# okieraised/rs-face-detection-tflite

Measured on AMD Instinct MI355X. Metric: faces/sec at batch=256 (256x256 back-camera) per GPU, higher is better.
Workload: dtype f32

## Files before the change

rs-face-detection-tflite_amd/csrc/mstrip_kernels.hip:

```cpp
#include <hip/hip_runtime.h>

#include <algorithm>
#include <cstdint>
#include <cstdio>
#include <cstdlib>
#include <type_traits>
#include <utility>

#include "kernels.hpp"
#include "launch.hpp"
#include "wave_sync.hpp"

namespace mi {

namespace {

typedef float v2f __attribute__((ext_vector_type(2)));
typedef float f32x4 __attribute__((ext_vector_type(4)));

struct MstripArgs {
    const float* in;
    float* out;
    const float* consts;
    long in_fs, out_fs;
    int B, H;
    int bands, band_rows;
    int has_res;
    float hi;
    unsigned long long* stamps;
};

constexpr int kMstripChain = 8;
struct MstripChainArgs {
    const float* in[kMstripChain];
    float* out[kMstripChain];
    const float* consts[kMstripChain];
    long in_fs[kMstripChain], out_fs[kMstripChain];
    int has_res[kMstripChain];
    float hi[kMstripChain];
    int nblocks, B, H;
};

template <int CK>
struct MK {
    static constexpr int C = 4 * CK, MT = C / 16;
    static constexpr int QP = CK + 1;
    static constexpr int PS = 4 * QP;
    static constexpr int IMG_F = 34 * PS;
    static constexpr int DPX = 64 / QP;
    static constexpr int NLD = 32 / DPX;
    static_assert(32 % DPX == 0 && NLD == 8, "eight DMA instructions per row (two source bases, four immediate offsets each)");
    static_assert((16 * PS) % 64 == 0 && 16 * PS / 64 < 256, "ds_read2st64_b32 reaches the second pixel tile");
    static constexpr int OFF_A = 0, A_F = CK * MT * 64, OFF_TAP = A_F, TAP_F = CK * 48, OFF_BIAS = OFF_TAP + TAP_F, OFF_SLOPE = OFF_BIAS + C, TOTAL = OFF_SLOPE + C;
    static constexpr int WG_F = A_F + 2 * C + TAP_F;
    static constexpr int NBUF = 2;
};

template <class F, int... KS>
__device__ __forceinline__ void mfor_each(F&& f, std::integer_sequence<int, KS...>) { (f(std::integral_constant<int, KS>{}), ...); }

template <int CK, bool RELU>
__global__ __launch_bounds__(256, 2) void mstrip_kernel(MstripArgs a) {
    using K = MK<CK>;
    constexpr int C = K::C, MT = K::MT, PS = K::PS, QP = K::QP, IMG_F = K::IMG_F, NLD = K::NLD, NBUF = K::NBUF;
    extern __shared__ __attribute__((aligned(16))) float lds[];
#ifdef MI_MSTRIP_STAMPS
    unsigned long long st_acc[7] = {0, 0, 0, 0, 0, 0, 0}, st_prev = __builtin_amdgcn_s_memtime();
#define MI_MSTAMP(k) { __builtin_amdgcn_sched_barrier(0); unsigned long long t_ = __builtin_amdgcn_s_memtime(); asm volatile("s_waitcnt lgkmcnt(0)" ::: "memory"); st_acc[k] += t_ - st_prev; st_prev = t_; __builtin_amdgcn_sched_barrier(0); }
#else
#define MI_MSTAMP(k)
#endif
    const int lane = threadIdx.x & 63;
    const int wave = __builtin_amdgcn_readfirstlane(threadIdx.x >> 6);
    const int kq = lane >> 4, p = lane & 15;
    float* wgc = lds;
    float* img = lds + K::WG_F + wave * NBUF * IMG_F;
    const int unit = blockIdx.x * 4 + wave;
    const int band = unit / a.B, b = unit - band * a.B;
    const bool active = band < a.bands;
    const int y0 = band * a.band_rows, y1 = min(y0 + a.band_rows, a.H);
    const float* in = a.in + (long)b * a.in_fs;

    const int goff = ((lane / QP) * C + 4 * min(lane % QP, CK - 1)) * 4;
    const unsigned lds_img = __builtin_amdgcn_readfirstlane((unsigned)(uintptr_t)(__attribute__((address_space(3))) float*)img);
    auto issue_row = [&](int r, int bi) {
        const char* src = reinterpret_cast<const char*>(in + (long)min(max(r, 0), a.H - 1) * 32 * C);
        const char* src1 = src + (NLD / 2) * K::DPX * C * 4;
        const unsigned dstb = lds_img + (unsigned)((bi * IMG_F + PS) * 4);
        constexpr int ACTIVE = K::DPX * QP;
        static_assert(ACTIVE > 32 && ACTIVE < 64, "exec mask written as two 32-bit halves");
        unsigned long long saved;
#define MI_MS_DMA(base, k) "s_add_u32 m0, m0, %7\n\ts_nop 0\n\tglobal_load_lds_dwordx4 %3, " base " offset:" #k "*%8\n\t"
        asm volatile("s_mov_b64 %0, exec\n\ts_mov_b32 exec_lo, -1\n\ts_mov_b32 exec_hi, %6\n\t"
                     "s_mov_b32 m0, %4\n\ts_nop 0\n\tglobal_load_lds_dwordx4 %3, %1\n\t"
                     MI_MS_DMA("%1", 1) MI_MS_DMA("%1", 2) MI_MS_DMA("%1", 3)
                     "s_add_u32 m0, m0, %5\n\ts_nop 0\n\tglobal_load_lds_dwordx4 %3, %2\n\t"
                     MI_MS_DMA("%2", 1) MI_MS_DMA("%2", 2) MI_MS_DMA("%2", 3)
                     "s_mov_b64 exec, %0"
                     : "=&s"(saved)
                     : "s"(src), "s"(src1), "v"(goff), "s"(dstb), "n"((NLD / 2) * K::DPX * PS * 4 - (NLD / 2 - 1) * K::DPX * (PS - C) * 4),
                       "n"((1u << (ACTIVE - 32)) - 1), "n"(K::DPX * (PS - C) * 4), "n"(K::DPX * C * 4)
                     : "memory", "scc", "m0");
#undef MI_MS_DMA
    };
    auto fix_row = [&](int r, int bi) {
        if (r >= 0 && r < a.H) return;
        float zz = 0.f;
        asm volatile("" : "+v"(zz));
        const float4 z = make_float4(zz, zz, zz, zz);
        float* part = img + bi * IMG_F + PS;
        constexpr int N4 = 32 * QP;
#pragma unroll
        for (int k = 0; k < (N4 + 63) / 64; k++)
            if (64 * (k + 1) <= N4 || lane < N4 - 64 * k) *reinterpret_cast<float4*>(part + 4 * (lane + 64 * k)) = z;
    };
    if (lane < 2 * QP) {
        const int col = lane / QP, qd = lane - col * QP;
#pragma unroll
        for (int bi = 0; bi < NBUF; bi++) *reinterpret_cast<float4*>(img + bi * IMG_F + col * 33 * PS + 4 * qd) = make_float4(0.f, 0.f, 0.f, 0.f);
    }

    if (active) issue_row(y0 - 1, 0);
    MI_MSTAMP(5)
    for (int i = threadIdx.x; i < K::A_F / 4; i += 256) reinterpret_cast<float4*>(wgc)[i] = reinterpret_cast<const float4*>(a.consts + K::OFF_A)[i];
    for (int i = threadIdx.x; i < 2 * C; i += 256) wgc[K::A_F + i] = a.consts[K::OFF_BIAS + i];
    for (int i = threadIdx.x; i < K::TAP_F / 4; i += 256) reinterpret_cast<float4*>(wgc + K::A_F + 2 * C)[i] = reinterpret_cast<const float4*>(a.consts + K::OFF_TAP)[i];
    if (active) issue_row(y0, 1);
    if (active) wait_vm<NLD>(); else wait_vm<0>();
    MI_MSTAMP(6)
    asm volatile("s_waitcnt lgkmcnt(0)" ::: "memory");
    __builtin_amdgcn_s_barrier();
    asm volatile("" ::: "memory");
    float tap[CK][9];
    {
        const float4* tp = reinterpret_cast<const float4*>(wgc + K::A_F + 2 * C) + kq * 3;
#pragma unroll
        for (int ks = 0; ks < CK; ks++) {
            const float4 t0 = tp[ks * 12], t1 = tp[ks * 12 + 1], t2 = tp[ks * 12 + 2];
            tap[ks][0] = t0.x; tap[ks][1] = t0.y; tap[ks][2] = t0.z; tap[ks][3] = t0.w;
            tap[ks][4] = t1.x; tap[ks][5] = t1.y; tap[ks][6] = t1.z; tap[ks][7] = t1.w;
            tap[ks][8] = t2.x;
        }
#pragma unroll
        for (int ks = 0; ks < CK; ks++)
#pragma unroll
            for (int t = 0; t < 9; t++) asm volatile("" : "+v"(tap[ks][t]));
    }
    if (!active) return;
    MI_MSTAMP(0)
    const float* xme = img + p * PS + kq;
    const float* sme = img + (1 + p) * PS + 4 * kq;
    const float* ame = wgc + lane;
    const unsigned ooff = (unsigned)(p * C + 4 * kq) * 4u;

    float accA[CK][2], accB[CK][2];
    f32x4 D[MT][2];
#pragma unroll
    for (int ks = 0; ks < CK; ks++) accA[ks][0] = accA[ks][1] = accB[ks][0] = accB[ks][1] = 0.f;

    auto init_D = [&](int bi) {
        float4 bs[MT], x[MT][2];
#pragma unroll
        for (int mt = 0; mt < MT; mt++) bs[mt] = *reinterpret_cast<const float4*>(wgc + K::A_F + 16 * mt + 4 * kq);
        if (a.has_res) {
#pragma unroll
            for (int mt = 0; mt < MT; mt++)
#pragma unroll
                for (int nt = 0; nt < 2; nt++) x[mt][nt] = *reinterpret_cast<const float4*>(sme + bi * IMG_F + 16 * nt * PS + 16 * mt);
#pragma unroll
            for (int mt = 0; mt < MT; mt++)
#pragma unroll
                for (int nt = 0; nt < 2; nt++) D[mt][nt] = f32x4{x[mt][nt].x + bs[mt].x, x[mt][nt].y + bs[mt].y, x[mt][nt].z + bs[mt].z, x[mt][nt].w + bs[mt].w};
        } else {
#pragma unroll
            for (int mt = 0; mt < MT; mt++) D[mt][0] = D[mt][1] = f32x4{bs[mt].x, bs[mt].y, bs[mt].z, bs[mt].w};
        }
    };
    typedef __attribute__((address_space(1))) char gchar;
    typedef __attribute__((address_space(1))) f32x4 gf32x4;
    auto epilogue = [&](int y) {
        gchar* dst = (gchar*)(a.out + (long)b * a.out_fs + (long)y * 32 * C);
        asm volatile("" : "+s"(dst));
#pragma unroll
        for (int mt = 0; mt < MT; mt++) {
            float4 sl = make_float4(0.f, 0.f, 0.f, 0.f);
            if (!RELU) sl = *reinterpret_cast<const float4*>(wgc + K::A_F + C + 16 * mt + 4 * kq);
#pragma unroll
            for (int nt = 0; nt < 2; nt++) {
                f32x4 v = D[mt][nt];
                if (RELU) {
                    v = f32x4{fmaxf(v.x, 0.f), fmaxf(v.y, 0.f), fmaxf(v.z, 0.f), fmaxf(v.w, 0.f)};
                } else {
                    v = f32x4{fminf(fmaxf(v.x, 0.f) + sl.x * fminf(v.x, 0.f), a.hi), fminf(fmaxf(v.y, 0.f) + sl.y * fminf(v.y, 0.f), a.hi),
                              fminf(fmaxf(v.z, 0.f) + sl.z * fminf(v.z, 0.f), a.hi), fminf(fmaxf(v.w, 0.f) + sl.w * fminf(v.w, 0.f), a.hi)};
                }
                *(gf32x4*)(dst + ooff + (unsigned)((16 * nt * C + 16 * mt) * 4)) = v;
            }
        }
    };

    const unsigned x_lds = (unsigned)(uintptr_t)(__attribute__((address_space(3))) float*)const_cast<float*>(xme);
    const unsigned a_lds = (unsigned)(uintptr_t)(__attribute__((address_space(3))) float*)const_cast<float*>(ame);
    auto row = [&](auto emit, int bi, float (&aPN)[CK][2], float (&aC)[CK][2]) {
        constexpr bool EMIT = decltype(emit)::value;
        const unsigned xr = x_lds + (unsigned)(bi * IMG_F * 4), ar = a_lds;
        float xs[2][3][2], av[2][MT];
        auto load_ks = [&](auto ksc, float (&x)[3][2], float (&aw)[MT]) {
            constexpr int ks = decltype(ksc)::value;
            const unsigned xa = xr, aa = ar;
#pragma unroll
            for (int dx = 0; dx < 3; dx++) {
                asm volatile("ds_read_b32 %0, %1 offset:%2" : "=v"(x[dx][0]) : "v"(xa), "n"((dx * PS + 4 * ks) * 4));
                asm volatile("ds_read_b32 %0, %1 offset:%2" : "=v"(x[dx][1]) : "v"(xa), "n"((dx * PS + 4 * ks + 16 * PS) * 4));
            }
            if constexpr (EMIT) {
#pragma unroll
                for (int mt = 0; mt < MT; mt++) asm volatile("ds_read_b32 %0, %1 offset:%2" : "=v"(aw[mt]) : "v"(aa), "n"((ks * MT + mt) * 64 * 4));
            }
        };
        auto landed = [&](float (&x)[3][2], float (&aw)[MT]) {
#pragma unroll
            for (int dx = 0; dx < 3; dx++) asm volatile("" : "+v"(x[dx][0]), "+v"(x[dx][1]));
            if constexpr (EMIT) {
#pragma unroll
                for (int mt = 0; mt < MT; mt++) asm volatile("" : "+v"(aw[mt]));
            }
        };
        auto kstep = [&](auto ksc) {
            constexpr int ks = decltype(ksc)::value;
            if constexpr (ks + 1 < CK) load_ks(std::integral_constant<int, ks + 1>{}, xs[(ks + 1) & 1], av[(ks + 1) & 1]);
            float (&x)[3][2] = xs[ks & 1];
            float (&aw)[MT] = av[ks & 1];
            const float (&w)[9] = tap[ks];
            float pch[2];
#pragma unroll
            for (int nt = 0; nt < 2; nt++) {
                float n = x[0][nt] * w[0], c = aC[ks][nt], pc = aPN[ks][nt];
#pragma unroll
                for (int dx = 0; dx < 3; dx++) {
                    if (EMIT) pc = __builtin_fmaf(x[dx][nt], w[6 + dx], pc);
                    if (dx) n = __builtin_fmaf(x[dx][nt], w[dx], n);
                    c = __builtin_fmaf(x[dx][nt], w[3 + dx], c);
                }
                aC[ks][nt] = c;
                aPN[ks][nt] = n;
                asm volatile("" : "+v"(aC[ks][nt]), "+v"(aPN[ks][nt]));
                pch[nt] = pc;
            }
            if constexpr (EMIT) {
#pragma unroll
                for (int mt = 0; mt < MT; mt++) {
                    D[mt][0] = __builtin_amdgcn_mfma_f32_16x16x4f32(aw[mt], pch[0], D[mt][0], 0, 0, 0);
                    D[mt][1] = __builtin_amdgcn_mfma_f32_16x16x4f32(aw[mt], pch[1], D[mt][1], 0, 0, 0);
                }
            }
            asm volatile("s_waitcnt lgkmcnt(0)" ::: "memory");
            if constexpr (ks + 1 < CK) landed(xs[(ks + 1) & 1], av[(ks + 1) & 1]);
            __builtin_amdgcn_sched_barrier(0);
        };
        load_ks(std::integral_constant<int, 0>{}, xs[0], av[0]);
        asm volatile("s_waitcnt lgkmcnt(0)" ::: "memory");
        landed(xs[0], av[0]);
        __builtin_amdgcn_sched_barrier(0);
        mfor_each(kstep, std::make_integer_sequence<int, CK>{});
    };

    constexpr int NST = 2 * MT;
    auto wait_row = [&](int t) {
        const bool st = t - 1 >= 2, dm = t == 0 || (t - 1) + 2 <= (y1 - y0 + 1);
        if (st && dm) wait_vm<NST + NLD>();
        else if (dm) wait_vm<NLD>();
        else if (st) wait_vm<NST>();
        else wait_vm<0>();
    };
    auto step = [&](auto emit, int r, float (&aPN)[CK][2], float (&aC)[CK][2]) {
        const int t = r - (y0 - 1), bi = t & 1;
        wait_row(t);
        fix_row(r, bi);
        wave_sync();
        MI_MSTAMP(1)
        row(emit, bi, aPN, aC);
        MI_MSTAMP(2)
        __builtin_amdgcn_sched_barrier(0);
        if constexpr (decltype(emit)::value) epilogue(r - 1);
        MI_MSTAMP(3)
        __builtin_amdgcn_sched_barrier(0);
        init_D(bi);
        __builtin_amdgcn_sched_barrier(0);
        wave_sync();
        __builtin_amdgcn_s_waitcnt(0xC07F);
        if (r + 2 <= y1) issue_row(r + 2, bi);
        MI_MSTAMP(4)
    };
    step(std::false_type{}, y0 - 1, accA, accB);
    step(std::false_type{}, y0, accB, accA);
    for (int r = y0 + 1; r <= y1; r += 2) {
        step(std::true_type{}, r, accA, accB);
        if (r + 1 > y1) break;
        step(std::true_type{}, r + 1, accB, accA);
    }
#ifdef MI_MSTRIP_STAMPS
    if (a.stamps && lane == 0)
        for (int k = 0; k < 7; k++) a.stamps[(long)unit * 8 + k] = st_acc[k];
#endif
}

template <int CK, bool RELU>
__global__ __launch_bounds__(512, 2) void mstrip_chain_kernel(MstripChainArgs ca) {
    using K = MK<CK>;
    constexpr int C = K::C, MT = K::MT, PS = K::PS, QP = K::QP, IMG_F = K::IMG_F, NLD = K::NLD, NBUF = K::NBUF;
    extern __shared__ __attribute__((aligned(16))) float lds[];
#ifdef MI_MSTRIP_STAMPS
    unsigned long long st_acc[7] = {0, 0, 0, 0, 0, 0, 0}, st_prev = __builtin_amdgcn_s_memtime();
#define MI_MSTAMP(k) { __builtin_amdgcn_sched_barrier(0); unsigned long long t_ = __builtin_amdgcn_s_memtime(); asm volatile("s_waitcnt lgkmcnt(0)" ::: "memory"); st_acc[k] += t_ - st_prev; st_prev = t_; __builtin_amdgcn_sched_barrier(0); }
#else
#define MI_MSTAMP(k)
#endif
    const int lane = threadIdx.x & 63;
    const int wave = __builtin_amdgcn_readfirstlane(threadIdx.x >> 6);
    const int kq = lane >> 4, p = lane & 15;
    float* img = lds + 2 * K::WG_F + wave * NBUF * IMG_F;
    const int b = blockIdx.x;
    const int y0 = 4 * wave, y1 = y0 + 4;
    struct { int H; } a{ca.H};
    const float* in = nullptr;
    float* wgc = lds;

    const int goff = ((lane / QP) * C + 4 * min(lane % QP, CK - 1)) * 4;
    const unsigned lds_img = __builtin_amdgcn_readfirstlane((unsigned)(uintptr_t)(__attribute__((address_space(3))) float*)img);
    auto issue_row = [&](int r, int bi) {
        const char* src = reinterpret_cast<const char*>(in + (long)min(max(r, 0), a.H - 1) * 32 * C);
        const char* src1 = src + (NLD / 2) * K::DPX * C * 4;
        const unsigned dstb = lds_img + (unsigned)((bi * IMG_F + PS) * 4);
        constexpr int ACTIVE = K::DPX * QP;
        static_assert(ACTIVE > 32 && ACTIVE < 64, "exec mask written as two 32-bit halves");
        unsigned long long saved;
#define MI_MS_DMA(base, k) "s_add_u32 m0, m0, %7\n\ts_nop 0\n\tglobal_load_lds_dwordx4 %3, " base " offset:" #k "*%8\n\t"
        asm volatile("s_mov_b64 %0, exec\n\ts_mov_b32 exec_lo, -1\n\ts_mov_b32 exec_hi, %6\n\t"
                     "s_mov_b32 m0, %4\n\ts_nop 0\n\tglobal_load_lds_dwordx4 %3, %1\n\t"
                     MI_MS_DMA("%1", 1) MI_MS_DMA("%1", 2) MI_MS_DMA("%1", 3)
                     "s_add_u32 m0, m0, %5\n\ts_nop 0\n\tglobal_load_lds_dwordx4 %3, %2\n\t"
                     MI_MS_DMA("%2", 1) MI_MS_DMA("%2", 2) MI_MS_DMA("%2", 3)
                     "s_mov_b64 exec, %0"
                     : "=&s"(saved)
                     : "s"(src), "s"(src1), "v"(goff), "s"(dstb), "n"((NLD / 2) * K::DPX * PS * 4 - (NLD / 2 - 1) * K::DPX * (PS - C) * 4),
                       "n"((1u << (ACTIVE - 32)) - 1), "n"(K::DPX * (PS - C) * 4), "n"(K::DPX * C * 4)
                     : "memory", "scc", "m0");
#undef MI_MS_DMA
    };
    auto fix_row = [&](int r, int bi) {
        if (r >= 0 && r < a.H) return;
        float zz = 0.f;
        asm volatile("" : "+v"(zz));
        const float4 z = make_float4(zz, zz, zz, zz);
        float* part = img + bi * IMG_F + PS;
        constexpr int N4 = 32 * QP;
#pragma unroll
        for (int k = 0; k < (N4 + 63) / 64; k++)
            if (64 * (k + 1) <= N4 || lane < N4 - 64 * k) *reinterpret_cast<float4*>(part + 4 * (lane + 64 * k)) = z;
    };
    if (lane < 2 * QP) {
        const int col = lane / QP, qd = lane - col * QP;
#pragma unroll
        for (int bi = 0; bi < NBUF; bi++) *reinterpret_cast<float4*>(img + bi * IMG_F + col * 33 * PS + 4 * qd) = make_float4(0.f, 0.f, 0.f, 0.f);
    }

    for (int i = threadIdx.x; i < K::A_F / 4; i += 512) reinterpret_cast<float4*>(wgc)[i] = reinterpret_cast<const float4*>(ca.consts[0] + K::OFF_A)[i];
    for (int i = threadIdx.x; i < 2 * C; i += 512) wgc[K::A_F + i] = ca.consts[0][K::OFF_BIAS + i];
    for (int i = threadIdx.x; i < K::TAP_F / 4; i += 512) reinterpret_cast<float4*>(wgc + K::A_F + 2 * C)[i] = reinterpret_cast<const float4*>(ca.consts[0] + K::OFF_TAP)[i];
  for (int blk = 0; blk < ca.nblocks; blk++) {
    wgc = lds + (blk & 1) * K::WG_F;
    in = ca.in[blk] + (long)b * ca.in_fs[blk];
    const int has_res = ca.has_res[blk];
    const float hi = ca.hi[blk];
    float* const outp = ca.out[blk] + (long)b * ca.out_fs[blk];
    issue_row(y0 - 1, 0);
    constexpr int NPRE = (K::WG_F / 4 + 511) / 512;
    float4 pre[NPRE];
    const bool more = blk + 1 < ca.nblocks;
    if (more) {
        const float* cn = ca.consts[blk + 1];
#pragma unroll
        for (int k = 0; k < NPRE; k++) {
            const int i = threadIdx.x + 512 * k;
            const int src = i < K::A_F / 4 ? K::OFF_A + 4 * i : (i < (K::A_F + 2 * C) / 4 ? K::OFF_BIAS + 4 * i - K::A_F : K::OFF_TAP + 4 * i - K::A_F - 2 * C);
            pre[k] = i < K::WG_F / 4 ? *reinterpret_cast<const float4*>(cn + src) : make_float4(0.f, 0.f, 0.f, 0.f);
        }
    }
    issue_row(y0, 1);
    wait_vm<NLD>();
    asm volatile("s_waitcnt lgkmcnt(0)" ::: "memory");
    if (blk == 0) {
        __builtin_amdgcn_s_barrier();
        asm volatile("" ::: "memory");
    }
    float tap[CK][9];
    {
        const float4* tp = reinterpret_cast<const float4*>(wgc + K::A_F + 2 * C) + kq * 3;
#pragma unroll
        for (int ks = 0; ks < CK; ks++) {
            const float4 t0 = tp[ks * 12], t1 = tp[ks * 12 + 1], t2 = tp[ks * 12 + 2];
            tap[ks][0] = t0.x; tap[ks][1] = t0.y; tap[ks][2] = t0.z; tap[ks][3] = t0.w;
            tap[ks][4] = t1.x; tap[ks][5] = t1.y; tap[ks][6] = t1.z; tap[ks][7] = t1.w;
            tap[ks][8] = t2.x;
        }
#pragma unroll
        for (int ks = 0; ks < CK; ks++)
#pragma unroll
            for (int t = 0; t < 9; t++) asm volatile("" : "+v"(tap[ks][t]));
    }
    MI_MSTAMP(0)
    const float* xme = img + p * PS + kq;
    const float* sme = img + (1 + p) * PS + 4 * kq;
    const float* ame = wgc + lane;
    const unsigned ooff = (unsigned)(p * C + 4 * kq) * 4u;

    float accA[CK][2], accB[CK][2];
    f32x4 D[MT][2];
#pragma unroll
    for (int ks = 0; ks < CK; ks++) accA[ks][0] = accA[ks][1] = accB[ks][0] = accB[ks][1] = 0.f;

    auto init_D = [&](int bi) {
        float4 bs[MT], x[MT][2];
#pragma unroll
        for (int mt = 0; mt < MT; mt++) bs[mt] = *reinterpret_cast<const float4*>(wgc + K::A_F + 16 * mt + 4 * kq);
        if (has_res) {
#pragma unroll
            for (int mt = 0; mt < MT; mt++)
#pragma unroll
                for (int nt = 0; nt < 2; nt++) x[mt][nt] = *reinterpret_cast<const float4*>(sme + bi * IMG_F + 16 * nt * PS + 16 * mt);
#pragma unroll
            for (int mt = 0; mt < MT; mt++)
#pragma unroll
                for (int nt = 0; nt < 2; nt++) D[mt][nt] = f32x4{x[mt][nt].x + bs[mt].x, x[mt][nt].y + bs[mt].y, x[mt][nt].z + bs[mt].z, x[mt][nt].w + bs[mt].w};
        } else {
#pragma unroll
            for (int mt = 0; mt < MT; mt++) D[mt][0] = D[mt][1] = f32x4{bs[mt].x, bs[mt].y, bs[mt].z, bs[mt].w};
        }
    };
    typedef __attribute__((address_space(1))) char gchar;
    typedef __attribute__((address_space(1))) f32x4 gf32x4;
    auto epilogue = [&](int y) {
        gchar* dst = (gchar*)(outp + (long)y * 32 * C);
        asm volatile("" : "+s"(dst));
#pragma unroll
        for (int mt = 0; mt < MT; mt++) {
            float4 sl = make_float4(0.f, 0.f, 0.f, 0.f);
            if (!RELU) sl = *reinterpret_cast<const float4*>(wgc + K::A_F + C + 16 * mt + 4 * kq);
#pragma unroll
            for (int nt = 0; nt < 2; nt++) {
                f32x4 v = D[mt][nt];
                if (RELU) {
                    v = f32x4{fmaxf(v.x, 0.f), fmaxf(v.y, 0.f), fmaxf(v.z, 0.f), fmaxf(v.w, 0.f)};
                } else {
                    v = f32x4{fminf(fmaxf(v.x, 0.f) + sl.x * fminf(v.x, 0.f), hi), fminf(fmaxf(v.y, 0.f) + sl.y * fminf(v.y, 0.f), hi),
                              fminf(fmaxf(v.z, 0.f) + sl.z * fminf(v.z, 0.f), hi), fminf(fmaxf(v.w, 0.f) + sl.w * fminf(v.w, 0.f), hi)};
                }
                *(gf32x4*)(dst + ooff + (unsigned)((16 * nt * C + 16 * mt) * 4)) = v;
            }
        }
    };

    const unsigned x_lds = (unsigned)(uintptr_t)(__attribute__((address_space(3))) float*)const_cast<float*>(xme);
    const unsigned a_lds = (unsigned)(uintptr_t)(__attribute__((address_space(3))) float*)const_cast<float*>(ame);
    auto row = [&](auto emit, int bi, float (&aPN)[CK][2], float (&aC)[CK][2]) {
        constexpr bool EMIT = decltype(emit)::value;
        const unsigned xr = x_lds + (unsigned)(bi * IMG_F * 4), ar = a_lds;
        float xs[2][3][2], av[2][MT];
        auto load_ks = [&](auto ksc, float (&x)[3][2], float (&aw)[MT]) {
            constexpr int ks = decltype(ksc)::value;
            const unsigned xa = xr, aa = ar;
#pragma unroll
            for (int dx = 0; dx < 3; dx++) {
                asm volatile("ds_read_b32 %0, %1 offset:%2" : "=v"(x[dx][0]) : "v"(xa), "n"((dx * PS + 4 * ks) * 4));
                asm volatile("ds_read_b32 %0, %1 offset:%2" : "=v"(x[dx][1]) : "v"(xa), "n"((dx * PS + 4 * ks + 16 * PS) * 4));
            }
            if constexpr (EMIT) {
#pragma unroll
                for (int mt = 0; mt < MT; mt++) asm volatile("ds_read_b32 %0, %1 offset:%2" : "=v"(aw[mt]) : "v"(aa), "n"((ks * MT + mt) * 64 * 4));
            }
        };
        auto landed = [&](float (&x)[3][2], float (&aw)[MT]) {
#pragma unroll
            for (int dx = 0; dx < 3; dx++) asm volatile("" : "+v"(x[dx][0]), "+v"(x[dx][1]));
            if constexpr (EMIT) {
#pragma unroll
                for (int mt = 0; mt < MT; mt++) asm volatile("" : "+v"(aw[mt]));
            }
        };
        auto kstep = [&](auto ksc) {
            constexpr int ks = decltype(ksc)::value;
            if constexpr (ks + 1 < CK) load_ks(std::integral_constant<int, ks + 1>{}, xs[(ks + 1) & 1], av[(ks + 1) & 1]);
            float (&x)[3][2] = xs[ks & 1];
            float (&aw)[MT] = av[ks & 1];
            const float (&w)[9] = tap[ks];
            float pch[2];
#pragma unroll
            for (int nt = 0; nt < 2; nt++) {
                float n = x[0][nt] * w[0], c = aC[ks][nt], pc = aPN[ks][nt];
#pragma unroll
                for (int dx = 0; dx < 3; dx++) {
                    if (EMIT) pc = __builtin_fmaf(x[dx][nt], w[6 + dx], pc);
                    if (dx) n = __builtin_fmaf(x[dx][nt], w[dx], n);
                    c = __builtin_fmaf(x[dx][nt], w[3 + dx], c);
                }
                aC[ks][nt] = c;
                aPN[ks][nt] = n;
                asm volatile("" : "+v"(aC[ks][nt]), "+v"(aPN[ks][nt]));
                pch[nt] = pc;
            }
            if constexpr (EMIT) {
#pragma unroll
                for (int mt = 0; mt < MT; mt++) {
                    D[mt][0] = __builtin_amdgcn_mfma_f32_16x16x4f32(aw[mt], pch[0], D[mt][0], 0, 0, 0);
                    D[mt][1] = __builtin_amdgcn_mfma_f32_16x16x4f32(aw[mt], pch[1], D[mt][1], 0, 0, 0);
                }
            }
            asm volatile("s_waitcnt lgkmcnt(0)" ::: "memory");
            if constexpr (ks + 1 < CK) landed(xs[(ks + 1) & 1], av[(ks + 1) & 1]);
            __builtin_amdgcn_sched_barrier(0);
        };
        load_ks(std::integral_constant<int, 0>{}, xs[0], av[0]);
        asm volatile("s_waitcnt lgkmcnt(0)" ::: "memory");
        landed(xs[0], av[0]);
        __builtin_amdgcn_sched_barrier(0);
        mfor_each(kstep, std::make_integer_sequence<int, CK>{});
    };

    constexpr int NST = 2 * MT;
    auto wait_row = [&](int t) {
        const bool st = t - 1 >= 2, dm = t == 0 || (t - 1) + 2 <= (y1 - y0 + 1);
        if (st && dm) wait_vm<NST + NLD>();
        else if (dm) wait_vm<NLD>();
        else if (st) wait_vm<NST>();
        else wait_vm<0>();
    };
    auto step = [&](auto emit, int r, float (&aPN)[CK][2], float (&aC)[CK][2]) {
        const int t = r - (y0 - 1), bi = t & 1;
        wait_row(t);
        fix_row(r, bi);
        wave_sync();
        MI_MSTAMP(1)
        row(emit, bi, aPN, aC);
        MI_MSTAMP(2)
        __builtin_amdgcn_sched_barrier(0);
        if constexpr (decltype(emit)::value) epilogue(r - 1);
        MI_MSTAMP(3)
        __builtin_amdgcn_sched_barrier(0);
        init_D(bi);
        __builtin_amdgcn_sched_barrier(0);
        wave_sync();
        __builtin_amdgcn_s_waitcnt(0xC07F);
        if (r + 2 <= y1) issue_row(r + 2, bi);
        MI_MSTAMP(4)
    };
    step(std::false_type{}, y0 - 1, accA, accB);
    step(std::false_type{}, y0, accB, accA);
    for (int r = y0 + 1; r <= y1; r += 2) {
        step(std::true_type{}, r, accA, accB);
        if (r + 1 > y1) break;
        step(std::true_type{}, r + 1, accB, accA);
    }
    asm volatile("s_waitcnt vmcnt(0)" ::: "memory");
    if (more) {
        float* nx = lds + ((blk + 1) & 1) * K::WG_F;
#pragma unroll
        for (int k = 0; k < NPRE; k++) {
            const int i = threadIdx.x + 512 * k;
            if (i < K::WG_F / 4) reinterpret_cast<float4*>(nx)[i] = pre[k];
        }
    }
    asm volatile("s_waitcnt vmcnt(0) lgkmcnt(0)" ::: "memory");
    __builtin_amdgcn_s_barrier();
    asm volatile("" ::: "memory");
  }
}

}

bool mstrip_shape_ok(int C, int Co) {
    static const bool off = getenv("MI_NO_MSTRIP") != nullptr;
    return !off && C == Co && C == 48;
}

bool mstrip_kernel_supports(const BlockArgs& a) {
    if (!a.w_strip || !a.has_dw || a.sh != 1 || a.sw != 1 || a.pt != 1 || a.pl != 1) return false;
    if (!mstrip_shape_ok(a.C, a.Co) || a.W != 32 || a.H != a.Ho || a.W != a.Wo || a.H < 2) return false;
    if (a.ep.res_mode != RES_NONE) {
        if (a.ep.res_after) return false;
        if (a.ep.res_mode != RES_DIRECT || a.ep.res != a.in || a.ep.res_fs != a.in_fs || a.ep.res_C != a.C) return false;
    }
    static const int min_b = getenv("MI_MSTRIP_MIN_B") ? atoi(getenv("MI_MSTRIP_MIN_B")) : 32;
    if (a.B < min_b) return false;
    auto aligned16 = [](const void* p) { return (reinterpret_cast<uintptr_t>(p) & 15) == 0; };
    return aligned16(a.in) && aligned16(a.out) && !(a.in_fs & 3) && !(a.out_fs & 3);
}

int mstrip_consts_floats(int C) { return C == 48 ? MK<12>::TOTAL : 0; }

void mstrip_pack_consts(int C, const float* w_dw, const float* b_dw, const float* w_pw, const float* bias, const float* alpha, int act, float* dst) {
    using K = MK<12>;
    std::fill(dst, dst + mstrip_consts_floats(C), 0.f);
    for (int ks = 0; ks < K::C / 4; ks++)
        for (int mt = 0; mt < K::MT; mt++)
            for (int l = 0; l < 64; l++) dst[K::OFF_A + (ks * K::MT + mt) * 64 + l] = w_pw[(size_t)(16 * mt + (l & 15)) * C + 4 * ks + (l >> 4)];
    for (int ks = 0; ks < K::C / 4; ks++)
        for (int kq = 0; kq < 4; kq++)
            for (int t = 0; t < 9; t++) dst[K::OFF_TAP + (ks * 4 + kq) * 12 + t] = w_dw[t * C + 4 * ks + kq];
    for (int c = 0; c < C; c++) {
        double acc = bias ? bias[c] : 0.0;
        if (b_dw)
            for (int k = 0; k < C; k++) acc += (double)w_pw[(size_t)c * C + k] * b_dw[k];
        dst[K::OFF_BIAS + c] = (float)acc;
        dst[K::OFF_SLOPE + c] = act == ACT_PRELU ? alpha[c] : (act == ACT_NONE ? 1.f : 0.f);
    }
}

const char* mstrip_kernel_label(const BlockArgs& a, char* buf, size_t cap) {
    snprintf(buf, cap, "mstrip_kernel<%d,%d>", a.C / 4, a.ep.act == ACT_RELU ? 1 : 0);
    return buf;
}

bool mstrip_chain_supports(const BlockArgs* blocks, int n) {
    static const bool off = getenv("MI_NO_MSTRIP_CHAIN") != nullptr;
    if (off || n < 2 || n > kMstripChain) return false;
    for (int k = 0; k < n; k++) {
        const BlockArgs& a = blocks[k];
        if (!mstrip_kernel_supports(a) || a.H != 32 || a.B != blocks[0].B || (a.ep.act == ACT_RELU) != (blocks[0].ep.act == ACT_RELU)) return false;
        if (k && a.in != blocks[k - 1].out) return false;
    }
    return true;
}

int launch_mstrip_chain(const BlockArgs* blocks, int n, void* stream) {
    using K = MK<12>;
    if (!mstrip_chain_supports(blocks, n)) return (int)hipErrorInvalidValue;
    MstripChainArgs ca{};
    ca.nblocks = n; ca.B = blocks[0].B; ca.H = blocks[0].H;
    for (int k = 0; k < n; k++) {
        const BlockArgs& a = blocks[k];
        ca.in[k] = a.in; ca.out[k] = a.out; ca.consts[k] = a.w_strip; ca.in_fs[k] = a.in_fs; ca.out_fs[k] = a.out_fs;
        ca.has_res[k] = a.ep.res_mode == RES_DIRECT;
        ca.hi[k] = a.ep.act == ACT_RELU6 ? 6.f : INFINITY;
    }
    const size_t lds_bytes = (size_t)(2 * K::WG_F + 8 * K::NBUF * K::IMG_F) * 4;
    const dim3 grid((unsigned)ca.B);
    hipStream_t s = (hipStream_t)stream;
    if (blocks[0].ep.act == ACT_RELU) {
        auto kern = mstrip_chain_kernel<12, true>;
        if (hipError_t e = allow_full_lds(reinterpret_cast<const void*>(kern)); e != hipSuccess) return (int)e;
        return (int)launch_kernel(kern, grid, dim3(512), lds_bytes, s, ca);
    }
    auto kern = mstrip_chain_kernel<12, false>;
    if (hipError_t e = allow_full_lds(reinterpret_cast<const void*>(kern)); e != hipSuccess) return (int)e;
    return (int)launch_kernel(kern, grid, dim3(512), lds_bytes, s, ca);
}

unsigned long long* g_mstrip_stamps = nullptr;

int launch_mstrip(const BlockArgs& a, void* stream) {
    using K = MK<12>;
    MstripArgs ma;
    ma.stamps = g_mstrip_stamps;
    ma.in = a.in; ma.out = a.out; ma.consts = a.w_strip; ma.in_fs = a.in_fs; ma.out_fs = a.out_fs;
    ma.B = a.B; ma.H = a.H;
    static const int forced = getenv("MI_MSTRIP_BAND") ? atoi(getenv("MI_MSTRIP_BAND")) : 0;
    long bands = std::max<long>(1, (8L * device_cu_count() + a.B / 2) / std::max(1, a.B));
    int rows = (int)((a.H + bands - 1) / bands);
    rows = std::max(rows, std::min(a.H, 4));
    if (forced > 0) rows = std::min(forced, a.H);
    ma.band_rows = rows;
    ma.bands = (a.H + rows - 1) / rows;
    ma.has_res = a.ep.res_mode == RES_DIRECT;
    ma.hi = a.ep.act == ACT_RELU6 ? 6.f : INFINITY;
    hipStream_t s = (hipStream_t)stream;
    const long units = (long)a.B * ma.bands;
    const size_t lds_bytes = (size_t)(K::WG_F + 4 * K::NBUF * K::IMG_F) * 4;
    const dim3 grid((unsigned)((units + 3) / 4));
    if (a.ep.act == ACT_RELU) {
        auto kern = mstrip_kernel<12, true>;
        if (hipError_t e = allow_full_lds(reinterpret_cast<const void*>(kern)); e != hipSuccess) return (int)e;
        return (int)launch_kernel(kern, grid, dim3(256), lds_bytes, s, ma);
    }
    auto kern = mstrip_kernel<12, false>;
    if (hipError_t e = allow_full_lds(reinterpret_cast<const void*>(kern)); e != hipSuccess) return (int)e;
    return (int)launch_kernel(kern, grid, dim3(256), lds_bytes, s, ma);
}

}
```

Measured before the change: 224,500.

## Restructure mstrip chain pipeline: specialised halo rows and cross-block row prefetch

The chain kernel's per-row loop is split into two specialised halo-row passes, which skip the MFMA and weight reads, and four emit steps. The last step skips the unused accumulator FMAs. The final emit step now issues the first row of the next chained block's input, so that load overlaps with the current block's tail. The prefetch of the next block's weights into registers moves after the first halo row. Per-wave timing stamps are added under a debug macro. The benefit depends on the more intricate buffer-parity and wait-count logic staying correct.

```diff
diff --git a/rs-face-detection-tflite_amd/csrc/mstrip_kernels.hip b/rs-face-detection-tflite_amd/csrc/mstrip_kernels.hip
--- a/rs-face-detection-tflite_amd/csrc/mstrip_kernels.hip
+++ b/rs-face-detection-tflite_amd/csrc/mstrip_kernels.hip
@@ -39,7 +39,11 @@
     int has_res[kMstripChain];
     float hi[kMstripChain];
     int nblocks, B, H;
+#ifdef MI_MSTRIP_STAMPS
+    unsigned* stamps;
+#endif
 };
+enum { CS_ISSUE, CS_TAPS, CS_ROW_WAIT, CS_HALO_WAIT, CS_HALO_ROWS, CS_HALO_TAIL, CS_EMIT_WAIT, CS_EMIT_ROWS, CS_EMIT_EPI, CS_EMIT_TAIL, CS_DRAIN, CS_HANDOFF, CS_BARRIER, kChainStamps = 16 };
 
 template <int CK>
 struct MK {
@@ -311,10 +315,11 @@
     constexpr int C = K::C, MT = K::MT, PS = K::PS, QP = K::QP, IMG_F = K::IMG_F, NLD = K::NLD, NBUF = K::NBUF;
     extern __shared__ __attribute__((aligned(16))) float lds[];
 #ifdef MI_MSTRIP_STAMPS
-    unsigned long long st_acc[7] = {0, 0, 0, 0, 0, 0, 0}, st_prev = __builtin_amdgcn_s_memtime();
-#define MI_MSTAMP(k) { __builtin_amdgcn_sched_barrier(0); unsigned long long t_ = __builtin_amdgcn_s_memtime(); asm volatile("s_waitcnt lgkmcnt(0)" ::: "memory"); st_acc[k] += t_ - st_prev; st_prev = t_; __builtin_amdgcn_sched_barrier(0); }
+    unsigned st_acc[kChainStamps] = {};
+    unsigned long long st_prev = __builtin_amdgcn_s_memtime();
+#define MI_CSTAMP(k) { __builtin_amdgcn_sched_barrier(0); unsigned long long t_ = __builtin_amdgcn_s_memtime(); asm volatile("s_waitcnt lgkmcnt(0)" ::: "memory"); st_acc[k] += (unsigned)(t_ - st_prev); st_prev = t_; __builtin_amdgcn_sched_barrier(0); }
 #else
-#define MI_MSTAMP(k)
+#define MI_CSTAMP(k)
 #endif
     const int lane = threadIdx.x & 63;
     const int wave = __builtin_amdgcn_readfirstlane(threadIdx.x >> 6);
@@ -323,13 +328,12 @@
     const int b = blockIdx.x;
     const int y0 = 4 * wave, y1 = y0 + 4;
     struct { int H; } a{ca.H};
-    const float* in = nullptr;
     float* wgc = lds;
 
     const int goff = ((lane / QP) * C + 4 * min(lane % QP, CK - 1)) * 4;
     const unsigned lds_img = __builtin_amdgcn_readfirstlane((unsigned)(uintptr_t)(__attribute__((address_space(3))) float*)img);
-    auto issue_row = [&](int r, int bi) {
-        const char* src = reinterpret_cast<const char*>(in + (long)min(max(r, 0), a.H - 1) * 32 * C);
+    auto issue_row = [&](const float* frame, int r, int bi) {
+        const char* src = reinterpret_cast<const char*>(frame + (long)min(max(r, 0), a.H - 1) * 32 * C);
         const char* src1 = src + (NLD / 2) * K::DPX * C * 4;
         const unsigned dstb = lds_img + (unsigned)((bi * IMG_F + PS) * 4);
         constexpr int ACTIVE = K::DPX * QP;
@@ -368,27 +372,24 @@
     for (int i = threadIdx.x; i < K::A_F / 4; i += 512) reinterpret_cast<float4*>(wgc)[i] = reinterpret_cast<const float4*>(ca.consts[0] + K::OFF_A)[i];
     for (int i = threadIdx.x; i < 2 * C; i += 512) wgc[K::A_F + i] = ca.consts[0][K::OFF_BIAS + i];
     for (int i = threadIdx.x; i < K::TAP_F / 4; i += 512) reinterpret_cast<float4*>(wgc + K::A_F + 2 * C)[i] = reinterpret_cast<const float4*>(ca.consts[0] + K::OFF_TAP)[i];
+    const float* xme = img + p * PS + kq;
+    const float* sme = img + (1 + p) * PS + 4 * kq;
+    const unsigned ooff = (unsigned)(p * C + 4 * kq) * 4u;
   for (int blk = 0; blk < ca.nblocks; blk++) {
     wgc = lds + (blk & 1) * K::WG_F;
-    in = ca.in[blk] + (long)b * ca.in_fs[blk];
+    const float* const in = ca.in[blk] + (long)b * ca.in_fs[blk];
     const int has_res = ca.has_res[blk];
     const float hi = ca.hi[blk];
     float* const outp = ca.out[blk] + (long)b * ca.out_fs[blk];
-    issue_row(y0 - 1, 0);
-    constexpr int NPRE = (K::WG_F / 4 + 511) / 512;
-    float4 pre[NPRE];
     const bool more = blk + 1 < ca.nblocks;
-    if (more) {
-        const float* cn = ca.consts[blk + 1];
-#pragma unroll
-        for (int k = 0; k < NPRE; k++) {
-            const int i = threadIdx.x + 512 * k;
-            const int src = i < K::A_F / 4 ? K::OFF_A + 4 * i : (i < (K::A_F + 2 * C) / 4 ? K::OFF_BIAS + 4 * i - K::A_F : K::OFF_TAP + 4 * i - K::A_F - 2 * C);
-            pre[k] = i < K::WG_F / 4 ? *reinterpret_cast<const float4*>(cn + src) : make_float4(0.f, 0.f, 0.f, 0.f);
-        }
-    }
-    issue_row(y0, 1);
-    wait_vm<NLD>();
+    const int ie = blk & 1, io = ie ^ 1;
+    issue_row(in, y0 - 1, ie);
+    if (blk == 0) issue_row(in, y0, io);
+    const float* ame = wgc + lane;
+
+    float accA[CK][2], accB[CK][2];
+    f32x4 D[MT][2];
+    MI_CSTAMP(CS_ISSUE)
     asm volatile("s_waitcnt lgkmcnt(0)" ::: "memory");
     if (blk == 0) {
         __builtin_amdgcn_s_barrier();
@@ -409,16 +410,7 @@
 #pragma unroll
             for (int t = 0; t < 9; t++) asm volatile("" : "+v"(tap[ks][t]));
     }
-    MI_MSTAMP(0)
-    const float* xme = img + p * PS + kq;
-    const float* sme = img + (1 + p) * PS + 4 * kq;
-    const float* ame = wgc + lane;
-    const unsigned ooff = (unsigned)(p * C + 4 * kq) * 4u;
-
-    float accA[CK][2], accB[CK][2];
-    f32x4 D[MT][2];
-#pragma unroll
-    for (int ks = 0; ks < CK; ks++) accA[ks][0] = accA[ks][1] = accB[ks][0] = accB[ks][1] = 0.f;
+    MI_CSTAMP(CS_TAPS)
 
     auto init_D = [&](int bi) {
         float4 bs[MT], x[MT][2];
@@ -463,8 +455,8 @@
 
     const unsigned x_lds = (unsigned)(uintptr_t)(__attribute__((address_space(3))) float*)const_cast<float*>(xme);
     const unsigned a_lds = (unsigned)(uintptr_t)(__attribute__((address_space(3))) float*)const_cast<float*>(ame);
-    auto row = [&](auto emit, int bi, float (&aPN)[CK][2], float (&aC)[CK][2]) {
-        constexpr bool EMIT = decltype(emit)::value;
+    auto row = [&](auto lastc, int bi, float (&aPN)[CK][2], float (&aC)[CK][2]) {
+        constexpr bool LAST = decltype(lastc)::value;
         const unsigned xr = x_lds + (unsigned)(bi * IMG_F * 4), ar = a_lds;
         float xs[2][3][2], av[2][MT];
         auto load_ks = [&](auto ksc, float (&x)[3][2], float (&aw)[MT]) {
@@ -475,18 +467,14 @@
                 asm volatile("ds_read_b32 %0, %1 offset:%2" : "=v"(x[dx][0]) : "v"(xa), "n"((dx * PS + 4 * ks) * 4));
                 asm volatile("ds_read_b32 %0, %1 offset:%2" : "=v"(x[dx][1]) : "v"(xa), "n"((dx * PS + 4 * ks + 16 * PS) * 4));
             }
-            if constexpr (EMIT) {
-#pragma unroll
-                for (int mt = 0; mt < MT; mt++) asm volatile("ds_read_b32 %0, %1 offset:%2" : "=v"(aw[mt]) : "v"(aa), "n"((ks * MT + mt) * 64 * 4));
-            }
+#pragma unroll
+            for (int mt = 0; mt < MT; mt++) asm volatile("ds_read_b32 %0, %1 offset:%2" : "=v"(aw[mt]) : "v"(aa), "n"((ks * MT + mt) * 64 * 4));
         };
         auto landed = [&](float (&x)[3][2], float (&aw)[MT]) {
 #pragma unroll
             for (int dx = 0; dx < 3; dx++) asm volatile("" : "+v"(x[dx][0]), "+v"(x[dx][1]));
-            if constexpr (EMIT) {
-#pragma unroll
-                for (int mt = 0; mt < MT; mt++) asm volatile("" : "+v"(aw[mt]));
-            }
+#pragma unroll
+            for (int mt = 0; mt < MT; mt++) asm volatile("" : "+v"(aw[mt]));
         };
         auto kstep = [&](auto ksc) {
             constexpr int ks = decltype(ksc)::value;
@@ -500,21 +488,21 @@
                 float n = x[0][nt] * w[0], c = aC[ks][nt], pc = aPN[ks][nt];
 #pragma unroll
                 for (int dx = 0; dx < 3; dx++) {
-                    if (EMIT) pc = __builtin_fmaf(x[dx][nt], w[6 + dx], pc);
-                    if (dx) n = __builtin_fmaf(x[dx][nt], w[dx], n);
-                    c = __builtin_fmaf(x[dx][nt], w[3 + dx], c);
+                    pc = __builtin_fmaf(x[dx][nt], w[6 + dx], pc);
+                    if (dx && !LAST) n = __builtin_fmaf(x[dx][nt], w[dx], n);
+                    if (!LAST) c = __builtin_fmaf(x[dx][nt], w[3 + dx], c);
                 }
-                aC[ks][nt] = c;
-                aPN[ks][nt] = n;
-                asm volatile("" : "+v"(aC[ks][nt]), "+v"(aPN[ks][nt]));
+                if constexpr (!LAST) {
+                    aC[ks][nt] = c;
+                    aPN[ks][nt] = n;
+                    asm volatile("" : "+v"(aC[ks][nt]), "+v"(aPN[ks][nt]));
+                }
                 pch[nt] = pc;
             }
-            if constexpr (EMIT) {
-#pragma unroll
-                for (int mt = 0; mt < MT; mt++) {
-                    D[mt][0] = __builtin_amdgcn_mfma_f32_16x16x4f32(aw[mt], pch[0], D[mt][0], 0, 0, 0);
-                    D[mt][1] = __builtin_amdgcn_mfma_f32_16x16x4f32(aw[mt], pch[1], D[mt][1], 0, 0, 0);
-                }
+#pragma unroll
+            for (int mt = 0; mt < MT; mt++) {
+                D[mt][0] = __builtin_amdgcn_mfma_f32_16x16x4f32(aw[mt], pch[0], D[mt][0], 0, 0, 0);
+                D[mt][1] = __builtin_amdgcn_mfma_f32_16x16x4f32(aw[mt], pch[1], D[mt][1], 0, 0, 0);
             }
             asm volatile("s_waitcnt lgkmcnt(0)" ::: "memory");
             if constexpr (ks + 1 < CK) landed(xs[(ks + 1) & 1], av[(ks + 1) & 1]);
@@ -526,42 +514,125 @@
         __builtin_amdgcn_sched_barrier(0);
         mfor_each(kstep, std::make_integer_sequence<int, CK>{});
     };
+    auto halo_row = [&](auto firstc, int bi, float (&aN)[CK][2], float (&aC)[CK][2], auto&& reads_done) {
+        constexpr bool FIRST = decltype(firstc)::value;
+        constexpr int G = FIRST ? CK : 4, NG = CK / G;
+        static_assert(CK % G == 0, "whole groups");
+        const unsigned xr = x_lds + (unsigned)(bi * IMG_F * 4);
+        float xg[NG > 1 ? 2 : 1][G][3][2];
+        auto load_g = [&](auto gc) {
+            constexpr int g = decltype(gc)::value;
+            mfor_each([&](auto jc) {
+                constexpr int j = decltype(jc)::value, ks = g * G + j;
+                float (&x)[3][2] = xg[g & 1][j];
+                const unsigned xa = xr;
+#pragma unroll
+                for (int dx = 0; dx < 3; dx++) {
+                    asm volatile("ds_read_b32 %0, %1 offset:%2" : "=v"(x[dx][0]) : "v"(xa), "n"((dx * PS + 4 * ks) * 4));
+                    asm volatile("ds_read_b32 %0, %1 offset:%2" : "=v"(x[dx][1]) : "v"(xa), "n"((dx * PS + 4 * ks + 16 * PS) * 4));
+                }
+            }, std::make_integer_sequence<int, G>{});
+        };
+        auto group = [&](auto gc) {
+            constexpr int g = decltype(gc)::value;
+            float (&x)[G][3][2] = xg[g & 1];
+            asm volatile("s_waitcnt lgkmcnt(0)" ::: "memory");
+#pragma unroll
+            for (int j = 0; j < G; j++)
+#pragma unroll
+                for (int dx = 0; dx < 3; dx++) asm volatile("" : "+v"(x[j][dx][0]), "+v"(x[j][dx][1]));
+            __builtin_amdgcn_sched_barrier(0);
+            if constexpr (g + 1 < NG) load_g(std::integral_constant<int, g + 1>{});
+            else reads_done();
+            __builtin_amdgcn_sched_barrier(0);
+#pragma unroll
+            for (int j = 0; j < G; j++) {
+                const float (&w)[9] = tap[g * G + j];
+#pragma unroll
+                for (int nt = 0; nt < 2; nt++) {
+                    float n = x[j][0][nt] * w[0];
+                    n = __builtin_fmaf(x[j][1][nt], w[1], n);
+                    n = __builtin_fmaf(x[j][2][nt], w[2], n);
+                    if constexpr (!FIRST) {
+                        float c = aC[g * G + j][nt];
+#pragma unroll
+                        for (int dx = 0; dx < 3; dx++) c = __builtin_fmaf(x[j][dx][nt], w[3 + dx], c);
+                        aC[g * G + j][nt] = c;
+                        asm volatile("" : "+v"(aC[g * G + j][nt]));
+                    }
+                    aN[g * G + j][nt] = n;
+                    asm volatile("" : "+v"(aN[g * G + j][nt]));
+                }
+            }
+            __builtin_amdgcn_sched_barrier(0);
+        };
+        load_g(std::integral_constant<int, 0>{});
+        mfor_each(group, std::make_integer_sequence<int, NG>{});
+    };
 
     constexpr int NST = 2 * MT;
-    auto wait_row = [&](int t) {
-        const bool st = t - 1 >= 2, dm = t == 0 || (t - 1) + 2 <= (y1 - y0 + 1);
-        if (st && dm) wait_vm<NST + NLD>();
-        else if (dm) wait_vm<NLD>();
-        else if (st) wait_vm<NST>();
-        else wait_vm<0>();
-    };
-    auto step = [&](auto emit, int r, float (&aPN)[CK][2], float (&aC)[CK][2]) {
-        const int t = r - (y0 - 1), bi = t & 1;
-        wait_row(t);
+    auto next_row = [&](const float* frame, int r, int bi) {
+        wave_sync();
+        __builtin_amdgcn_s_waitcnt(0xC07F);
+        issue_row(frame, r, bi);
+    };
+    if (blk == 0) wait_vm<NLD>(); else wait_vm<0>();
+    MI_CSTAMP(CS_ROW_WAIT)
+    fix_row(y0 - 1, ie);
+    wave_sync();
+    MI_CSTAMP(CS_HALO_WAIT)
+    halo_row(std::true_type{}, ie, accA, accB, [&] { next_row(in, y0 + 1, ie); });
+    MI_CSTAMP(CS_HALO_ROWS)
+    wait_vm<NLD>();
+    constexpr int NPRE = (K::WG_F / 4 + 511) / 512;
+    float4 pre[NPRE];
+    if (more) {
+        const float* cn = ca.consts[blk + 1];
+#pragma unroll
+        for (int k = 0; k < NPRE; k++) {
+            const int i = threadIdx.x + 512 * k;
+            const int src = i < K::A_F / 4 ? K::OFF_A + 4 * i : (i < (K::A_F + 2 * C) / 4 ? K::OFF_BIAS + 4 * i - K::A_F : K::OFF_TAP + 4 * i - K::A_F - 2 * C);
+            pre[k] = i < K::WG_F / 4 ? *reinterpret_cast<const float4*>(cn + src) : make_float4(0.f, 0.f, 0.f, 0.f);
+        }
+    }
+    wave_sync();
+    MI_CSTAMP(CS_HALO_WAIT)
+    halo_row(std::false_type{}, io, accB, accA, [] {});
+    MI_CSTAMP(CS_HALO_ROWS)
+    __builtin_amdgcn_sched_barrier(0);
+    init_D(io);
+    __builtin_amdgcn_sched_barrier(0);
+    next_row(in, y0 + 2, io);
+    MI_CSTAMP(CS_HALO_TAIL)
+    auto step = [&](auto lastc, int t, float (&aPN)[CK][2], float (&aC)[CK][2]) {
+        constexpr bool LAST = decltype(lastc)::value;
+        const int r = y0 - 1 + t, bi = t & 1 ? io : ie;
+        if (t == 2) wait_vm<NLD>();
+        else if (!LAST || more) wait_vm<NST + NLD>();
+        else wait_vm<NST>();
         fix_row(r, bi);
         wave_sync();
-        MI_MSTAMP(1)
-        row(emit, bi, aPN, aC);
-        MI_MSTAMP(2)
+        MI_CSTAMP(CS_EMIT_WAIT)
+        row(lastc, bi, aPN, aC);
+        MI_CSTAMP(CS_EMIT_ROWS)
         __builtin_amdgcn_sched_barrier(0);
-        if constexpr (decltype(emit)::value) epilogue(r - 1);
-        MI_MSTAMP(3)
-        __builtin_amdgcn_sched_barrier(0);
-        init_D(bi);
-        __builtin_amdgcn_sched_barrier(0);
-        wave_sync();
-        __builtin_amdgcn_s_waitcnt(0xC07F);
-        if (r + 2 <= y1) issue_row(r + 2, bi);
-        MI_MSTAMP(4)
-    };
-    step(std::false_type{}, y0 - 1, accA, accB);
-    step(std::false_type{}, y0, accB, accA);
-    for (int r = y0 + 1; r <= y1; r += 2) {
-        step(std::true_type{}, r, accA, accB);
-        if (r + 1 > y1) break;
-        step(std::true_type{}, r + 1, accB, accA);
-    }
+        epilogue(r - 1);
+        MI_CSTAMP(CS_EMIT_EPI)
+        if constexpr (!LAST) {
+            __builtin_amdgcn_sched_barrier(0);
+            init_D(bi);
+            __builtin_amdgcn_sched_barrier(0);
+            if (r + 2 <= y1) next_row(in, r + 2, bi);
+            else if (more) next_row(ca.in[blk + 1] + (long)b * ca.in_fs[blk + 1], y0, bi);
+            MI_CSTAMP(CS_EMIT_TAIL)
+        }
+    };
+    step(std::false_type{}, 2, accA, accB);
+    step(std::false_type{}, 3, accB, accA);
+    step(std::false_type{}, 4, accA, accB);
+    step(std::true_type{}, 5, accB, accA);
     asm volatile("s_waitcnt vmcnt(0)" ::: "memory");
+    MI_CSTAMP(CS_DRAIN)
     if (more) {
         float* nx = lds + ((blk + 1) & 1) * K::WG_F;
 #pragma unroll
@@ -571,8 +642,23 @@
         }
     }
     asm volatile("s_waitcnt vmcnt(0) lgkmcnt(0)" ::: "memory");
+    MI_CSTAMP(CS_HANDOFF)
     __builtin_amdgcn_s_barrier();
     asm volatile("" ::: "memory");
+    MI_CSTAMP(CS_BARRIER)
+#ifdef MI_MSTRIP_STAMPS
+    if (ca.stamps) {
+        unsigned* dst = ca.stamps + (((long)b * ca.nblocks + blk) * 8 + wave) * kChainStamps;
+#pragma unroll
+        for (int k = 0; k < kChainStamps; k++) {
+            if (lane == 0) dst[k] = st_acc[k];
+            st_acc[k] = 0;
+        }
+        asm volatile("s_waitcnt vmcnt(0)" ::: "memory");
+        st_prev = __builtin_amdgcn_s_memtime();
+        __builtin_amdgcn_s_waitcnt(0xC07F);
+    }
+#endif
   }
 }
 
@@ -632,11 +718,16 @@
     return true;
 }
 
+unsigned long long* g_mstrip_stamps = nullptr;
+
 int launch_mstrip_chain(const BlockArgs* blocks, int n, void* stream) {
     using K = MK<12>;
     if (!mstrip_chain_supports(blocks, n)) return (int)hipErrorInvalidValue;
     MstripChainArgs ca{};
     ca.nblocks = n; ca.B = blocks[0].B; ca.H = blocks[0].H;
+#ifdef MI_MSTRIP_STAMPS
+    ca.stamps = reinterpret_cast<unsigned*>(g_mstrip_stamps);
+#endif
     for (int k = 0; k < n; k++) {
         const BlockArgs& a = blocks[k];
         ca.in[k] = a.in; ca.out[k] = a.out; ca.consts[k] = a.w_strip; ca.in_fs[k] = a.in_fs; ca.out_fs[k] = a.out_fs;
@@ -655,8 +746,6 @@
     if (hipError_t e = allow_full_lds(reinterpret_cast<const void*>(kern)); e != hipSuccess) return (int)e;
     return (int)launch_kernel(kern, grid, dim3(512), lds_bytes, s, ca);
 }
-
-unsigned long long* g_mstrip_stamps = nullptr;
 
 int launch_mstrip(const BlockArgs& a, void* stream) {
     using K = MK<12>;
```

After: 225,900 (median of 6 runs). No clear change (+0.6%).
